# vladiant/CascadeClassifier

Measured on AMD Instinct MI355X. Metric: detection Mwindows/sec (1080p, haarcascade_frontalface) + achieved HBM GB/s, higher is better.
Workload: dtype i32+f32 (f64 stage sums)

## Files before the change

cascadeclassifier_amd/_lib.py:

```python
from __future__ import annotations

import ctypes as C
import os

_HERE = os.path.dirname(os.path.abspath(__file__))
LIB_PATH = os.environ.get("CCAMD_LIB") or os.path.join(_HERE, "lib", "libcascadeclassifier_amd.so")

CC_OK = 0
CC_ERR_INVALID_ARG = -1
CC_ERR_NO_DEVICE = -2
CC_ERR_HIP = -3
CC_ERR_IO = -4
CC_ERR_PARSE = -5
CC_ERR_UNSUPPORTED = -6
CC_ERR_BUFFER_TOO_SMALL = -7
CC_ERR_OUT_OF_RANGE = -8
CC_ERR_NO_TRAIN_PARAMS = -9

CC_FEATURE_HAAR, CC_FEATURE_LBP, CC_FEATURE_HOG = 0, 1, 2
CC_PIX_GRAY8, CC_PIX_BGR8, CC_PIX_BGRA8, CC_PIX_RGB8, CC_PIX_RGBA8, CC_PIX_RGB8_PLANAR = 0, 1, 2, 3, 4, 5
CC_HAAR_BASIC, CC_HAAR_CORE, CC_HAAR_ALL = 0, 1, 2


class CascadeError(RuntimeError):
# ... 119 lines not shown
    "cc_detect_batch_device_only": (_i, [_vp, _vp, _i, _i, _i, _i, _sz, _sz, C.POINTER(DetectParams)]),
    "cc_detect_multiscale_fmt": (_i, [_vp, _vp, _i, _i, _sz, _i, C.POINTER(DetectParams), _vp, _i, C.POINTER(_i)]),
    "cc_detect_batch_fmt": (_i, [_vp, _vp, _i, _i, _i, _i, _sz, _sz, _i, C.POINTER(DetectParams), _vp, _i, _vp]),
    "cc_detect_batch_submit_fmt": (_i, [_vp, _vp, _i, _i, _i, _i, _sz, _sz, _i, C.POINTER(DetectParams), _pp]),
    "cc_detect_batch_to_device": (_i, [_vp, _vp, _i, _i, _i, _i, _sz, _sz, _i, C.POINTER(DetectParams), _vp, _i, _vp,
                                       C.POINTER(_i)]),
    "cc_detect_batch_levels_fmt": (_i, [_vp, _vp, _i, _i, _i, _i, _sz, _sz, _i, C.POINTER(DetectParams), _vp, _vp, _vp, _i, _vp]),
    "cc_detect_batch_to_device_levels": (_i, [_vp, _vp, _i, _i, _i, _i, _sz, _sz, _i, C.POINTER(DetectParams), _vp, _vp, _vp, _i,
                                              _vp, C.POINTER(_i)]),
    "cc_detect_multiscale_levels_fmt": (_i, [_vp, _vp, _i, _i, _sz, _i, C.POINTER(DetectParams), _vp, _vp, _vp, _i,
                                             C.POINTER(_i)]),
    "cc_to_gray_u8": (_i, [_i, _vp, _i, _i, _i, _sz, _vp, _sz]),
    "cc_detect_multiscale_levels": (_i, [_vp, _vp, _i, _i, _sz, C.POINTER(DetectParams), _vp, _vp, _vp, _i, C.POINTER(_i)]),
    "cc_detect_raw": (_i, [_vp, _vp, _i, _i, _sz, C.POINTER(DetectParams), _vp, _i, C.POINTER(_i)]),
    "cc_detect_debug_windows": (_i, [_vp, _vp, _i, _i, _sz, C.POINTER(DetectParams), _vp, _vp, _vp, C.c_int64,
                                     C.POINTER(C.c_int64)]),
    "cc_scale_plan": (_i, [_i, _i, _i, _i, C.POINTER(DetectParams), _vp, _i, C.POINTER(_i)]),
    "cc_detector_specialize": (_i, [_vp, _i]),
    "cc_detector_specialize_async": (_i, [_vp, _i]),
    "cc_detector_specialized_stages": (_i, [_vp]),
    "cc_cascade_compile_specialized": (_i, [_vp, _i, C.c_char_p, C.POINTER(C.c_size_t)]),
    "cc_detector_set_profiling": (_i, [_vp, _i]),
    "cc_detector_graph_active": (_i, [_vp]),
    "cc_detector_graph_captures": (C.c_int64, [_vp]),
    "cc_detector_get_timings": (_i, [_vp, C.POINTER(DetectorTimings), _i]),
    "cc_detector_candidate_capacity": (_i, [_vp]),
    "cc_integral_u8": (_i, [_i, _vp, _i, _i, _sz, _vp, _vp, _vp]),
    "cc_resize_linear_exact_u8": (_i, [_i, _vp, _i, _i, _sz, _vp, _i, _i, _sz]),
    "cc_debug_stream_dwords": (_i, [_i, _sz, _i, C.POINTER(C.c_uint32)]),
    "cc_debug_division_check": (_i, [_i, C.c_uint64, C.c_uint64, C.POINTER(C.c_uint64)]),
    "cc_debug_vnf_check": (_i, [_i, C.c_uint64, C.c_uint64, C.POINTER(C.c_uint64)]),
    "cc_debug_wave_int_tables": (_i, [_vp, _vp, _vp, _vp, _vp]),
    "cc_debug_spec_step1_plan": (_i, [_vp, _i, _i, _vp, _vp, _vp, _vp]),
    "cc_group_rectangles": (_i, [_vp, _i, _i, _d, _vp, _i, C.POINTER(_i)]),
    "cc_group_rectangles_device": (_i, [_i, _vp, _vp, _i, _i, _d, _vp, _i, _vp, C.POINTER(_i)]),
    "cc_group_rectangles_levels": (_i, [_vp, _vp, _vp, _i, _i, _d, _vp, _vp, _vp, _i, C.POINTER(_i)]),
    "cc_group_rectangles_device_levels": (_i, [_i, _vp, _vp, _vp, _vp, _i, _i, _d, _vp, _vp, _vp, _i, _vp, C.POINTER(_i)]),
    "cc_eval_create": (_i, [_i, _i, _i, _i, _i, _i, _pp]),
    "cc_eval_destroy": (None, [_vp]),
    "cc_eval_num_features": (_i, [_vp]),
    "cc_eval_max_cat_count": (_i, [_vp]),
    "cc_eval_feature_size": (_i, [_vp]),
    "cc_eval_feature_geometry": (_i, [_vp, _i, _vp, _vp, C.POINTER(_i)]),
    "cc_eval_set_image": (_i, [_vp, _vp, _sz, C.c_uint8, _i]),
    "cc_eval_set_images": (_i, [_vp, _vp, _i, _i, _vp]),
    "cc_eval_labels": (C.POINTER(C.c_float), [_vp]),
    "cc_eval_calc": (_i, [_vp, _i, _i, C.POINTER(C.c_float)]),
    "cc_eval_calc_list": (_i, [_vp, _vp, _i, _i, _vp]),
    "cc_eval_calc_batch": (_i, [_vp, _i, _i, _vp, _i, _vp, _i]),
    "cc_eval_calc_batch_device": (_i, [_vp, _i, _i, _vp, _i, _vp, _sz]),
    "cc_eval_calc_batch_sorted": (_i, [_vp, _i, _i, _i, _vp, _vp, _i]),
    "cc_eval_calc_custom_haar": (_i, [_vp, _vp, _i, _i, _vp, _i, _vp]),
    "cc_haar_feature_calc": (_i, [_i, _vp, _i, _i, _vp, _vp, _i, _i, _vp]),
    "cc_eval_get_sample": (_i, [_vp, _i, _vp, _vp, _vp]),
    "cc_eval_hog_feature_geometry": (_i, [_vp, _i, _vp]),
    "cc_eval_get_hog_sample": (_i, [_vp, _i, _vp, _vp]),
    "cc_debug_hog_bins": (_i, [_i, C.POINTER(C.c_int32), _vp, _vp]),
    "cc_debug_hog_lds": (_i, [_i, _i, C.POINTER(_i), C.POINTER(_i), C.POINTER(C.c_int64), C.POINTER(C.c_int64)]),
    "cc_eval_predict_cascade": (_i, [_vp, _vp, _vp, _i, _vp]),
    "cc_eval_last_kernel_ms": (_i, [_vp, C.POINTER(C.c_double)]),
    "cc_debug_eval_tile_samples": (_i, [_vp]),
    "cc_eval_presort": (_i, [_vp, _i]),
    "cc_eval_presort_range": (_i, [_vp, _i, _i, _i]),
    "cc_presort_plan": (_i, [_i, _i, _i, C.c_uint64, C.POINTER(_i), C.POINTER(_i), C.POINTER(C.c_uint64)]),
    "cc_eval_presort_split": (_i, [_vp, _i, _i, _i, _i, _i]),
    "cc_eval_table_bytes": (_i, [_vp, C.POINTER(C.c_uint64)]),
# ... 98 lines not shown
```

cascadeclassifier_amd/csrc/cc_eval_common.h:

```cpp
#ifndef CC_EVAL_COMMON_H
#define CC_EVAL_COMMON_H

constexpr int TILE_X = 64;
#ifndef CC_TILE_Y
#define CC_TILE_Y 8
#endif
#ifndef CC_EVAL_THREADS
#define CC_EVAL_THREADS 256
#endif
#ifndef CC_EVAL_MIN_WAVES_PER_EU
#define CC_EVAL_MIN_WAVES_PER_EU 5
#endif
constexpr int TILE_Y = CC_TILE_Y;
constexpr int EVAL_THREADS = CC_EVAL_THREADS;
constexpr int EVAL_WAVES = EVAL_THREADS / 64;
constexpr int WIN_PER_THREAD = TILE_Y / EVAL_WAVES;
constexpr int SPEC_PARTS = EVAL_WAVES >= 8 ? 8 : EVAL_WAVES >= 4 ? 4 : EVAL_WAVES >= 2 ? 2 : 1;

struct ScaleDev {
  int w, h;
  int pitch8, pitchI;
  long long img_ofs, int_ofs, mask_ofs, win_ofs, h_ofs;
  int ystep, nx, ny, nxw, nbands;
  float scale;
  int win_w, win_h;
  int xtab_ofs, ytab_ofs;
};

struct HaarStumpDev {
  int ofs[3][4];
  float w[3];
  float thr, left, right;
  int nrect;
  int pad;
};
struct LbpStumpDev {
  int ofs[16];
  float left, right;
  int subset[8];
  int pad[2];
};

struct HaarNodeDev {
  int ofs[3][4];
  float w[3];
  float thr;
  int left, right;
  int nrect;
  int pad;
// ... 36 lines not shown

struct TileGeom16 {
  static constexpr bool k16 = true;
  int cols, rows, rs16, row_stride;
  __host__ __device__ TileGeom16(int W0, int H0, int tile_y = TILE_Y) {
    cols = (TILE_X - 1) * 2 + W0 + 1;
    rows = (tile_y - 1) * 2 + H0 + 1;
    rs16 = (cols + 3) / 4 * 4;
    if (rs16 % 16 == 0) rs16 += 4;
    row_stride = rs16 / 2;
  }
  __host__ __device__ int at(int r, int c) const { return r * rs16 + c; }
  __host__ __device__ int words() const { return rows * row_stride; }
};

constexpr int TILE_WINDOWS = TILE_X * TILE_Y;
constexpr int MAX_STAGES = 64;
constexpr int PART_DOUBLES = (EVAL_WAVES - 1) * 64;
constexpr int QUEUE_ROWS = TILE_WINDOWS / 32;
constexpr int VNF_PITCH = TILE_X + 32;
__host__ __device__ inline int tile_words_padded(int tile_words) { return (tile_words + 3) & ~3; }
__host__ __device__ inline size_t eval_lds_bytes(int tile_words, bool tilted, bool haar = true, int tile_y = TILE_Y, bool lean = false) {
  if (lean) return (size_t)tile_words_padded(tile_words) * 4 + tile_y * TILE_X * 4 + 2 * (tile_y * TILE_X) * 2 + 3 * 32 * 4;
  return (size_t)tile_words_padded(tile_words) * 4 * (tilted ? 2 : 1) + PART_DOUBLES * 8 + (haar ? tile_y * VNF_PITCH * 4 : 0) +
         2 * (tile_y * TILE_X) * 2 + 3 * 32 * 4;
}
__host__ __device__ inline int lean_split_gap_bytes(int tile_y, int rows) { return 2 * (tile_y * TILE_X) * 2 - 2 * rows * 32 * 2; }
__host__ __device__ inline int split_part_bytes(int ns) { return (ns - 1) * (EVAL_THREADS / ns) * 8; }
constexpr int CU_LDS_BYTES = 160 * 1024;
__host__ __device__ inline int lds_blocks_per_cu(size_t lds_bytes) {
  const int n = (int)((size_t)CU_LDS_BYTES / (lds_bytes ? lds_bytes : 1)), cap = 32 / EVAL_WAVES;
  return n > cap ? cap : n;
}

template <int CTRL, int ROW_MASK>
__device__ __forceinline__ double dpp_f64(double v) {
  const unsigned long long u = __double_as_longlong(v);
  const int lo = __builtin_amdgcn_update_dpp(0, (int)(unsigned)u, CTRL, ROW_MASK, 0xF, false);
  const int hi = __builtin_amdgcn_update_dpp(0, (int)(unsigned)(u >> 32), CTRL, ROW_MASK, 0xF, false);
  return __longlong_as_double(((unsigned long long)(unsigned)hi << 32) | (unsigned)lo);
}
__device__ __forceinline__ double readlane_f64(double v, int src) {
  const unsigned long long u = __double_as_longlong(v);
  const unsigned lo = __builtin_amdgcn_readlane((int)(unsigned)u, src);
  const unsigned hi = __builtin_amdgcn_readlane((int)(unsigned)(u >> 32), src);
  return __longlong_as_double(((unsigned long long)hi << 32) | lo);
}
__device__ __forceinline__ double wave_sum_f64(double v) {
  v += dpp_f64<0xB1, 0xF>(v);
  v += dpp_f64<0x4E, 0xF>(v);
  v += dpp_f64<0x141, 0xF>(v);
  v += dpp_f64<0x140, 0xF>(v);
  v += dpp_f64<0x142, 0xA>(v);
  v += dpp_f64<0x143, 0xC>(v);
  return readlane_f64(v, 63);
}
__device__ __forceinline__ int lane_rank(unsigned long long mask) {
  return __builtin_amdgcn_mbcnt_hi((unsigned)(mask >> 32), __builtin_amdgcn_mbcnt_lo((unsigned)mask, 0));
}

#endif
```

cascadeclassifier_amd/csrc/cc_eval_kernel.inc:

```

#define CC_CONST __attribute__((address_space(4)))
template <class T>
__device__ __forceinline__ const T CC_CONST* as_const_table(const T* p) {
  return (const T CC_CONST*)p;
}
template <class T>
__device__ __forceinline__ T load_record(const T CC_CONST* p) {
  static_assert(sizeof(T) % 4 == 0, "table records are dword multiples");
  T out;
  const int CC_CONST* w = (const int CC_CONST*)p;
  int* o = reinterpret_cast<int*>(&out);
#pragma unroll
  for (unsigned i = 0; i < sizeof(T) / 4; i++) o[i] = w[i];
  return out;
}

constexpr int STAGE_ROWS = 12;
template <int STEP, class Geom>
__device__ __forceinline__ void stage_tile(int32_t* lds, const Geom& G, const int32_t* __restrict__ sum,
                                           const ScaleDev& S, int x0, int y0) {
  const int lane = threadIdx.x & 63, wave = __builtin_amdgcn_readfirstlane(threadIdx.x >> 6);
  const int quads = (G.cols + 3) >> 2;
  const bool right_edge = x0 + quads * 4 - 1 > S.w;
  for (int q0 = 0; q0 < quads; q0 += 64) {
// ... 245 lines not shown

struct QueueState {
  int qg = 1;
  int st = 1;
  int n = 0, rows = 0, my_rows = 0;
};
struct WaveShare {
  int cnt, my_id;
  unsigned long long alive;
};

template <int STEP, bool HAAR, bool TREES>
struct EvalTile {
  using Stump = typename cc_select<HAAR, HaarStumpDev, LbpStumpDev>::type;
  using Node = typename cc_select<HAAR, HaarNodeDev, LbpNodeDev>::type;
#ifdef CC_SPEC_TILE16
  static constexpr bool G16 = STEP == 2 && !TREES;
#else
  static constexpr bool G16 = false;
#endif
  using Geom = typename cc_select<G16, TileGeom16, TileGeom<STEP>>::type;

  const EvalArgs& A;
  int32_t* const lds;
  const int4 T;
  const ScaleDev& S;
#ifdef CC_SPEC_W0
  static constexpr int W0 = CC_SPEC_W0, H0 = CC_SPEC_H0;
#else
  const int W0 = A.W0, H0 = A.H0;
#endif
  const Geom G{W0, H0};
#ifdef CC_LEAN_LDS
  static constexpr bool kLean = HAAR && !TREES && STEP == 1;
#else
  static constexpr bool kLean = false;
#endif
  double* const s_part = kLean ? nullptr : reinterpret_cast<double*>(lds + tile_words_padded(G.words()) * ((HAAR && A.tilt_chan >= 0) ? 2 : 1));
  float* const s_vnf = kLean ? reinterpret_cast<float*>(lds + tile_words_padded(G.words())) : reinterpret_cast<float*>(s_part + PART_DOUBLES);
  unsigned short* const s_q = reinterpret_cast<unsigned short*>(s_vnf + (HAAR ? TILE_Y * (kLean ? TILE_X : VNF_PITCH) : 0));
  int* const s_cnt = reinterpret_cast<int*>(s_q + 2 * TILE_WINDOWS);
  const int frame = blockIdx.y;
  const int32_t* const sum = A.integ + ((size_t)frame * A.nchan + 0) * A.int_frame_elems + S.int_ofs;
  const int lane = threadIdx.x & 63, wave = __builtin_amdgcn_readfirstlane(threadIdx.x >> 6);
  const int half = lane >> 5, cls = lane & 31;
  const int gx0 = T.y * TILE_X, gy0 = T.z * TILE_Y;
  const int skew = (STEP * G.row_stride) & 31;
  const Node* const nodes = reinterpret_cast<const Node*>(STEP == 2 ? A.nodes2 : A.nodes1);
  const Stump CC_CONST* const stumps = as_const_table(reinterpret_cast<const Stump*>(G16 ? A.gstumps : STEP == 2 ? A.stumps2 : A.stumps1));
  const int CC_CONST* const stage_first = as_const_table(A.stage_first);
  const int CC_CONST* const stage_ntrees = as_const_table(A.stage_ntrees);
  const float CC_CONST* const stage_thr = as_const_table(A.stage_thr);
  const int CC_CONST* const group_first = as_const_table(A.group_first);
  const double CC_CONST* const wave_q = as_const_table(A.wave_q);
  const int CC_CONST* const wave_thr_q = as_const_table(A.wave_thr_q);
  const bool dbg = A.dbg_codes != nullptr && frame == 0;

  __device__ __forceinline__ EvalTile(const EvalArgs& A_, int32_t* lds_, const int4 T_, const ScaleDev& S_) : A(A_), lds(lds_), T(T_), S(S_) {}

  __device__ __forceinline__ void stamp(int slot) const {
    if (A.stamps && threadIdx.x == 0)
      A.stamps[((size_t)blockIdx.y * gridDim.x + blockIdx.x) * STAMP_SLOTS + slot] = __builtin_amdgcn_s_memtime();
  }
  __device__ __forceinline__ int window_base(int id) const { return ((id >> 6) * STEP) * G.row_stride + (id & 63); }
  __device__ __forceinline__ auto table_reader(int id) const {
    if constexpr (G16)
      return GlobalReader{sum, (unsigned)((gy0 + (id >> 6)) * STEP) * (unsigned)S.pitchI + (unsigned)((gx0 + (id & 63)) * STEP), S.pitchI};
    else
      return LdsReader{lds + window_base(id)};
  }
  __device__ __forceinline__ void report(int id, int code, double last) const {
    const size_t o = (size_t)S.win_ofs + (size_t)(gy0 + (id >> 6)) * S.nx + (gx0 + (id & 63));
    A.dbg_codes[o] = code;
    if (A.dbg_sums) A.dbg_sums[o] = last;
  }
  __device__ __forceinline__ void emit_candidate(int id, double last_sum) const {
    const int slot = atomicAdd(A.cand_count, 1);
    if (slot < A.cand_cap) A.cands[slot] = CandRaw{frame, T.x, gx0 + (id & 63), gy0 + (id >> 6), last_sum};
  }
  __device__ __forceinline__ int win_class(int id) const { return ((id & 63) + skew * (id >> 6)) & 31; }
  __device__ __forceinline__ int vnf_slot(int id) const {
    if constexpr (kLean)
      return (id & ~63) | (((id & 63) + skew * (id >> 6)) & 63);
    else
      return (id >> 6) * (TILE_X + skew) + (id & 63);
  }
  __device__ __forceinline__ int q_index(int g, int row, int c) const {
    if constexpr (kLean)
      return (g & 1) ? (2 * QUEUE_ROWS - 1 - row) * 32 + c : row * 32 + c;
    else
      return (g & 1) * TILE_WINDOWS + row * 32 + c;
  }
// ... 100 lines not shown
        for (int j = lo; j < nt; j += step) {
          const Stump nxt = load_record(stumps + first + min(j + step, nt - 1));
          acc += stump_vote(rd, cur, vnf);
          cur = nxt;
        }
      }
    } else {
      for (int j = lo; j < nt; j += step) acc += stump_vote(rd, stumps + first + j, vnf);
    }
    return acc;
  }
  __device__ __forceinline__ WaveShare deal_windows(const QueueState& h) const {
    const unsigned short* q = s_q + (h.qg & 1) * TILE_WINDOWS;
    unsigned short* my_list = wave_lists(h.qg) + wave * 64;
    int numbered = 0;
    for (int r0 = 0; r0 < h.rows; r0 += 2) {
      const int row = r0 + half;
      const bool valid = row < h.my_rows;
      const int id = valid ? queued(q, h.qg, row, cls) : 0;
      const unsigned long long mask = __ballot(valid);
      const int number = numbered + lane_rank(mask);
      if (valid && number % EVAL_WAVES == wave) my_list[number / EVAL_WAVES] = (unsigned short)id;
      numbered += __builtin_popcountll(mask);
    }
    const int cnt = (numbered - wave + EVAL_WAVES - 1) / EVAL_WAVES;
    return WaveShare{cnt, lane < cnt ? my_list[lane] : 0, cnt >= 64 ? ~0ull : ((1ull << cnt) - 1ull)};
  }

  __device__ __forceinline__ void stage_phase(unsigned (&valsq_pre)[WIN_PER_THREAD]) const {
    unsigned sq_raw[WIN_PER_THREAD][4];
#pragma unroll
    for (int k = 0; k < WIN_PER_THREAD; k++) {
      sq_raw[k][0] = sq_raw[k][1] = sq_raw[k][2] = sq_raw[k][3] = 0;
      if (HAAR) {
        const int gx = min(gx0 + lane, S.nx - 1), gy = min(gy0 + wave * WIN_PER_THREAD + k, S.ny - 1);
        const unsigned* sq = reinterpret_cast<const unsigned*>(A.integ + ((size_t)frame * A.nchan + 1) * A.int_frame_elems + S.int_ofs);
        const int nrx = W0 - 2, nry = H0 - 2;
        size_t q0;
        int dx;
        if (STEP == 2 && A.sq_compact) {
          q0 = (size_t)(gy * 2 + 1) * S.pitchI + gx;
          dx = nrx >> 1;
        } else {
          q0 = (size_t)(gy * STEP + 1) * S.pitchI + (gx * STEP + 1);
          dx = nrx;
        }
        sq_raw[k][0] = sq[q0];
        sq_raw[k][1] = sq[q0 + dx];
        sq_raw[k][2] = sq[q0 + (size_t)nry * S.pitchI];
        sq_raw[k][3] = sq[q0 + (size_t)nry * S.pitchI + dx];
      }
    }
#ifdef CC_PRIO_STAGE
    __builtin_amdgcn_s_setprio(CC_PRIO_STAGE);
#endif
    stage_tile<STEP>(lds, G, sum, S, gx0 * STEP, gy0 * STEP);
    if (HAAR && A.tilt_chan >= 0)
      stage_tile<STEP>(lds + tile_words_padded(G.words()), G,
                       A.integ + ((size_t)frame * A.nchan + A.tilt_chan) * A.int_frame_elems + S.int_ofs, S, gx0 * STEP, gy0 * STEP);
    if (threadIdx.x < 3 * 32) s_cnt[threadIdx.x] = 0;
#pragma unroll
    for (int k = 0; k < WIN_PER_THREAD; k++) valsq_pre[k] = sq_raw[k][0] - sq_raw[k][1] - sq_raw[k][2] + sq_raw[k][3];
    __syncthreads();
#ifdef CC_PRIO_STAGE
    __builtin_amdgcn_s_setprio(0);
#endif
  }

  static constexpr bool kRolledDense = !HAAR && !TREES && WIN_PER_THREAD > 2;
  __device__ __forceinline__ void dense_phase_rolled() const {
    const int gx = gx0 + lane;
    const double thr0 = (double)stage_thr[0];
    unsigned long long* const mask_col = mask_column();
    [[maybe_unused]] const int nt0 = stage_ntrees[0];
#pragma unroll 1
    for (int k = 0; k < WIN_PER_THREAD; k++) {
      const int ly = wave * WIN_PER_THREAD + k;
      const int32_t* b = lds + (ly * STEP) * G.row_stride + lane;
      const bool alive = gx < S.nx && gy0 + ly < S.ny;
      double acc = 0.;
      if (__any(alive)) {
#ifdef CC_SPEC_STAGES
        acc = spec_stage<STEP>(0, 0, SPEC_PARTS, b, 1.f);
#else
        for (int i = 0; i < nt0; i++) acc += stump_vote(LdsReader{b}, stumps + i, 1.f);
#endif
      }
      deliver(stage0_outcome(ly, alive, acc, thr0, mask_col), ly * 64 + lane, acc, A.nstages == 1, 1);
    }
  }
  __device__ __forceinline__ bool dense_phase(const unsigned (&valsq_pre)[WIN_PER_THREAD]) const {
    int base[WIN_PER_THREAD];
    float vnf[WIN_PER_THREAD];
    bool alive[WIN_PER_THREAD];
    const int gx = gx0 + lane;
#pragma unroll
    for (int k = 0; k < WIN_PER_THREAD; k++) {
      const int ly = wave * WIN_PER_THREAD + k;
      const int gy = gy0 + ly;
      base[k] = (ly * STEP) * G.row_stride + lane;
      vnf[k] = 1.f;
      alive[k] = gx < S.nx && gy < S.ny;
      if (HAAR) {
        const bool in_grid = alive[k];
        alive[k] = false;
        if (in_grid) {
          const int nrx = W0 - 2, nry = H0 - 2;
          const double area = (double)(nrx * nry);
          const int32_t* b = lds + base[k];
          int valsum;
          if constexpr (G16) {
            const unsigned short* h = reinterpret_cast<const unsigned short*>(b);
            const int hx = nrx >> 1;
            const unsigned a0 = h[G.at(1, 1)], a1 = h[G.at(1, 1 + hx)], a2 = h[G.at(1, 1 + nrx)];
            const unsigned c0 = h[G.at(1 + nry, 1)], c1 = h[G.at(1 + nry, 1 + hx)], c2 = h[G.at(1 + nry, 1 + nrx)];
            valsum = (int)(((a0 - a1 - c0 + c1) & 0xffffu) + ((a1 - a2 - c1 + c2) & 0xffffu));
          } else
            valsum = b[G.at(1, 1)] - b[G.at(1, 1 + nrx)] - b[G.at(1 + nry, 1)] + b[G.at(1 + nry, 1 + nrx)];
          const unsigned valsq = valsq_pre[k];
          double nf = area * (double)valsq - (double)valsum * (double)valsum;
          if (nf > 0.) {
            vnf[k] = inv_sqrt_as_float(nf);
            alive[k] = area * (double)vnf[k] < 1e-1;
          }
          if (dbg && !alive[k]) report(ly * 64 + lane, -1, 0.0);
        }
      }
    }
    if (A.stop_after == -3) {
      float sink = 0;
#pragma unroll
      for (int k = 0; k < WIN_PER_THREAD; k++) sink += alive[k] ? vnf[k] : 0.f;
      if (HAAR && sink == 12345.f) s_vnf[0] = sink;
      return false;
    }
    bool any_mine = false;
    double acc[WIN_PER_THREAD];
#pragma unroll
    for (int k = 0; k < WIN_PER_THREAD; k++) {
      any_mine |= alive[k];
      acc[k] = 0.;
    }
    if (__any(any_mine)) {
      [[maybe_unused]] const int nt = stage_ntrees[0];
      if constexpr (TREES) {
        for (int i = 0; i < nt; i++) {
          const int root = as_const_table(A.tree_root)[i], leaf0 = as_const_table(A.tree_leaf0)[i];
#pragma unroll
          for (int k = 0; k < WIN_PER_THREAD; k++)
            if (alive[k]) acc[k] += tree_vote(lds + base[k], nodes, root, leaf0, A.leaves, vnf[k]);
        }
      } else {
#ifdef CC_SPEC_STAGES
        if constexpr (WIN_PER_THREAD == 2) {
          spec_stage0_x2<STEP>(lds + base[0], lds + base[1], vnf[0], vnf[1], acc[0], acc[1]);
        } else {
#pragma unroll
          for (int k = 0; k < WIN_PER_THREAD; k++) acc[k] = spec_stage<STEP>(0, 0, SPEC_PARTS, lds + base[k], vnf[k]);
        }
#else
        if constexpr (HAAR) {
          Stump cur = load_record(stumps);
          for (int i = 0; i < nt; i++) {
            const Stump nxt = load_record(stumps + min(i + 1, nt - 1));
#pragma unroll
            for (int k = 0; k < WIN_PER_THREAD; k++) acc[k] += stump_vote(LdsReader{lds + base[k]}, cur, vnf[k]);
            cur = nxt;
          }
        } else {
          for (int i = 0; i < nt; i++) {
#pragma unroll
            for (int k = 0; k < WIN_PER_THREAD; k++) acc[k] += stump_vote(LdsReader{lds + base[k]}, stumps + i, vnf[k]);
          }
        }
#endif
      }
    }
    const double thr = (double)stage_thr[0];
    unsigned long long* const mask_col = mask_column();
    bool pass_k[WIN_PER_THREAD];
#pragma unroll
    for (int k = 0; k < WIN_PER_THREAD; k++) pass_k[k] = stage0_outcome(wave * WIN_PER_THREAD + k, alive[k], acc[k], thr, mask_col);
    const bool last_group = A.nstages == 1;
#pragma unroll
    for (int k = 0; k < WIN_PER_THREAD; k++) {
      const int id = (wave * WIN_PER_THREAD + k) * 64 + lane;
      if (HAAR && pass_k[k] && !last_group) s_vnf[vnf_slot(id)] = vnf[k];
      deliver(pass_k[k], id, acc[k], last_group, 1);
    }
    return true;
  }

  __device__ __forceinline__ bool thread_phase(QueueState& h) const {
    for (; h.qg < A.ngroups; h.qg++) {
      const int qg = h.qg;
      const int st = h.st = group_first[qg];
      const int st_end = group_first[qg + 1];
      if (A.stop_after >= 0 && st > A.stop_after) return false;
      __syncthreads();
      if (qg >= A.dense_from) {
        h.n = min(s_cnt[(qg % 3) * 32], TILE_WINDOWS);
        h.rows = (h.n + 31) >> 5;
        h.my_rows = max(0, (h.n - cls + 31) >> 5);
      } else {
        h.my_rows = min(s_cnt[(qg % 3) * 32 + cls], QUEUE_ROWS);
        h.rows = wave_max_u32(h.my_rows);
        h.n = wave_sum_u32(h.my_rows) >> 1;
      }
      if (threadIdx.x < 32) s_cnt[((qg + 2) % 3) * 32 + threadIdx.x] = 0;
      if (st + 2 < STAMP_SLOTS - 1) stamp(st + 2);
      if (h.n == 0 || h.n < A.wave_below) break;
      const unsigned short* q = s_q + (qg & 1) * TILE_WINDOWS;
      const bool last_group = st_end >= A.nstages;
      const int groups = (h.rows + 1) >> 1;
      const bool may_split = A.split_stumps && st_end - st == 1;
      const int g_split = may_split ? groups - groups % EVAL_WAVES : groups;
      const int rem = groups - g_split;
      int ns = 1;
      if (rem > 0)
// ... 243 lines not shown
```

cascadeclassifier_amd/csrc/cc_spec.hip:

```cpp
#include <hip/hip_runtime.h>

#include <algorithm>
#include <array>
#include <cmath>
#include <cstdlib>
#include <cstring>
#include <map>
#include <mutex>

#include <dlfcn.h>
#include <sys/stat.h>
#include <unistd.h>

#include "cc_detect_internal.h"

namespace ccamd {

#include "build/cc_eval_kernel_src.h"

struct SpecStump {
  std::string loads;
  std::string decls;
  std::string compute;
  double base = 0.;
// ... 490 lines not shown
  bool ok() const { return create && compile && log_size && log && code_size && code && destroy; }
};

static const HipRtcApi& hiprtc_api() {
  static HipRtcApi api;
  static std::once_flag once;
  std::call_once(once, [] {
    for (const char* name : {"libhiprtc.so.7", "libhiprtc.so", "/opt/rocm/lib/libhiprtc.so"}) {
      api.lib = dlopen(name, RTLD_NOW | RTLD_LOCAL);
      if (api.lib) break;
    }
    if (!api.lib) return;
    auto sym = [&](const char* n) { return dlsym(api.lib, n); };
    api.create = reinterpret_cast<decltype(api.create)>(sym("hiprtcCreateProgram"));
    api.compile = reinterpret_cast<decltype(api.compile)>(sym("hiprtcCompileProgram"));
    api.log_size = reinterpret_cast<decltype(api.log_size)>(sym("hiprtcGetProgramLogSize"));
    api.log = reinterpret_cast<decltype(api.log)>(sym("hiprtcGetProgramLog"));
    api.code_size = reinterpret_cast<decltype(api.code_size)>(sym("hiprtcGetCodeSize"));
    api.code = reinterpret_cast<decltype(api.code)>(sym("hiprtcGetCode"));
    api.destroy = reinterpret_cast<decltype(api.destroy)>(sym("hiprtcDestroyProgram"));
    api.version = reinterpret_cast<decltype(api.version)>(sym("hiprtcVersion"));
  });
  return api;
}

static const char kSpecPrelude[] =
    "typedef signed char int8_t;\ntypedef unsigned char uint8_t;\ntypedef short int16_t;\ntypedef unsigned short uint16_t;\n"
    "typedef int int32_t;\ntypedef unsigned int uint32_t;\ntypedef long long int64_t;\ntypedef unsigned long long uint64_t;\n";

struct SpecModulePlan {
  int only_step, tile_y;
};
static bool spec_lean_lds(const Cascade& m, int tmode, int only_step) {
  return only_step == 1 && tmode == TILE_32 && m.feature_type == CC_FEATURE_HAAR && !m.has_tilted;
}
static size_t spec_step1_lds(const Cascade& m, int tile_y) {
  return eval_lds_bytes(TileGeom<1>(m.win_w, m.win_h, tile_y).words(), false, true, tile_y, true);
}
constexpr int kSpecStep1Rows = 20;
constexpr int kSpecStep1MinBlocks = 4;
static int spec_step1_rows(const Cascade& m, int want) {
  int ty = want;
  while (ty - EVAL_WAVES >= TILE_Y && lds_blocks_per_cu(spec_step1_lds(m, ty)) < kSpecStep1MinBlocks) ty -= EVAL_WAVES;
  return ty;
}
constexpr int kStep1WaveBelow = 32;
int spec_wave_below(int detector_value, int only_step, int tile_y) {
  if (only_step != 1 || detector_value <= 0) return -1;
  if (const char* e = std::getenv("CCAMD_WAVE_BELOW1")) return std::max(0, std::min(64, std::atoi(e)));
  if (std::getenv("CCAMD_WAVE_BELOW") || tile_y < 12) return -1;
  return std::max(detector_value, kStep1WaveBelow);
}

static std::vector<SpecModulePlan> spec_modules(const Cascade& m, int tmode) {
  auto valid = [&](int ty) { return ty >= EVAL_WAVES && ty <= 32 && ty % EVAL_WAVES == 0; };
  auto env_rows = [&](const char* name, int dflt) {
    const char* e = std::getenv(name);
    const int v = e ? std::atoi(e) : dflt;
    return valid(v) ? v : dflt;
  };
  if (m.has_tilted) return {{0, TILE_Y}};
  const bool lbp16 = m.feature_type == CC_FEATURE_LBP && tmode == TILE_16;
  const bool haar32 = tmode == TILE_32 && m.feature_type == CC_FEATURE_HAAR;
  const bool rows_given = std::getenv("CCAMD_SPEC_TILE_Y") != nullptr;
  const int all = env_rows("CCAMD_SPEC_TILE_Y", lbp16 ? 20 : TILE_Y);
  const bool two = (haar32 || std::getenv("CCAMD_SPEC_TWO_MODULES")) && !std::getenv("CCAMD_SPEC_ONE_MODULE");
  if (!two) return {{0, all}};
  return {{2, env_rows("CCAMD_SPEC_TILE_Y2", all)}, {1, env_rows("CCAMD_SPEC_TILE_Y1", (haar32 && !rows_given) ? spec_step1_rows(m, kSpecStep1Rows) : all)}};
}

static cc_status compile_specialised(const std::string& src, const std::string& arch, int n_stages, bool lbp, int tmode, int tile_y, int only_step, int win_w, int win_h,
                                     int lean_blocks, std::vector<char>& code) {
  const bool tile16 = tmode == TILE_16;
  static std::mutex mu;
  static std::map<std::string, std::vector<char>> cache;
  const std::string o_arch = "--offload-arch=" + arch, o_k = "-DCC_SPEC_STAGES=" + std::to_string(n_stages);
  const std::string o_ty = "-DCC_TILE_Y=" + std::to_string(tile_y), o_th = "-DCC_EVAL_THREADS=" + std::to_string(EVAL_THREADS);
  int min_waves = tile16 ? (tile_y >= 20 ? 6 : 7) : CC_EVAL_MIN_WAVES_PER_EU;
  if (lean_blocks > 0) {
    min_waves = std::max(1, std::min(8, lean_blocks * EVAL_WAVES / 4));
    if (const char* e = std::getenv("CCAMD_SPEC_WAVES1")) min_waves = std::max(1, std::min(8, std::atoi(e)));
  }
  const std::string o_w = "-DCC_EVAL_MIN_WAVES_PER_EU=" + std::to_string(min_waves);
  const std::string o_step = "-DCC_ONLY_STEP=" + std::to_string(only_step);
  const std::string o_w0 = "-DCC_SPEC_W0=" + std::to_string(win_w), o_h0 = "-DCC_SPEC_H0=" + std::to_string(win_h);
  std::vector<const char*> optv = {o_arch.c_str(), "-O3", "-std=c++17", "-ffp-contract=off", "-fno-fast-math", o_k.c_str(), o_ty.c_str(), o_th.c_str(), o_w.c_str(), o_w0.c_str(), o_h0.c_str()};
  if (only_step) optv.push_back(o_step.c_str());
  if (lbp) optv.push_back("-DCC_SPEC_LBP");
  if (tile16) optv.push_back("-DCC_SPEC_TILE16");
  if (lean_blocks > 0) optv.push_back("-DCC_LEAN_LDS");
  const char* const* opts = optv.data();
  const int n_opts = (int)optv.size();
  std::string key;
  {
    int major = 0, minor = 0;
    const HipRtcApi& rtc = hiprtc_api();
    if (rtc.version) (void)rtc.version(&major, &minor);
    key += "hiprtc " + std::to_string(major) + "." + std::to_string(minor) + " ";
  }
  for (int i = 0; i < n_opts; i++) key += std::string(opts[i]) + " ";
  key += "#" + src;
  {
    std::lock_guard<std::mutex> lk(mu);
    auto it = cache.find(key);
    if (it != cache.end()) {
      code = it->second;
      return CC_OK;
    }
  }
  struct CacheHeader {
    char magic[8];
    unsigned long long key_len, h1, h2;
  };
  auto hash_key = [&](unsigned long long seed, unsigned long long prime) {
// ... 81 lines not shown
      const bool ok = std::fwrite(&want, sizeof(want), 1, f) == 1 && std::fwrite(code.data(), 1, code.size(), f) == code.size();
      std::fclose(f);
      if (!ok || std::rename(tmp.c_str(), cache_file.c_str()) != 0) (void)std::remove(tmp.c_str());
    }
  }
  std::lock_guard<std::mutex> lk(mu);
  cache[key] = code;
  return CC_OK;
}

cc_status spec_build(const Cascade& m, int n_stages, const std::string& arch, std::vector<SpecCode>& codes, int& k_out, int& tmode_out) {
  if (cc_status hs = refuse_hog(m, "cc_detector_specialize"); hs != CC_OK) return hs;
  if (m.max_nodes_per_tree > 1) return set_error(CC_ERR_UNSUPPORTED, "cc_detector_specialize: stump cascades only");
  int k = 0, stumps = 0;
  const int budget = 320;
  while (k < (int)m.stage_ntrees.size() && k < n_stages && k < MAX_STAGES && (k == 0 || stumps + m.stage_ntrees[(size_t)k] <= budget))
    stumps += m.stage_ntrees[(size_t)k++];
  std::string src = kSpecPrelude;
  src += "namespace ccamd {\n";
  src += kEvalKernelSrc;
  src += "\n}  // namespace ccamd\n";
  const std::string marker = "//@@CC_SPEC_FUNCTIONS@@";
  const size_t pos = src.find(marker);
  if (pos == std::string::npos) return set_error(CC_ERR_HIP, "cc_detector_specialize: kernel source has no specialisation marker");
  const int tmode = tile16_eligible(m, k) ? TILE_16 : TILE_32;
  src.replace(pos, marker.size(), spec_stage_source(m, k, tmode));
  k_out = k;
  tmode_out = tmode;
  codes.clear();
  for (const SpecModulePlan& mp : spec_modules(m, tmode)) {
    SpecCode c;
    c.only_step = mp.only_step;
    c.tile_y = mp.tile_y;
    const int lean_blocks = spec_lean_lds(m, tmode, mp.only_step) ? std::max(1, lds_blocks_per_cu(spec_step1_lds(m, mp.tile_y))) : 0;
    const cc_status st = compile_specialised(src, arch, k, m.feature_type == CC_FEATURE_LBP, tmode, mp.tile_y, mp.only_step, m.win_w, m.win_h, lean_blocks, c.code);
    if (st != CC_OK) return st;
    codes.push_back(std::move(c));
  }
  return CC_OK;
}

cc_status spec_load(const Cascade& m, const std::vector<SpecCode>& codes, int tmode, size_t base_lds, SpecModule out[2], int* n_out) {
  if (codes.empty() || codes.size() > 2) return set_error(CC_ERR_HIP, "cc_detector_specialize: %zu modules", codes.size());
  const bool haar_k = m.feature_type == CC_FEATURE_HAAR;
  int n = 0;
  auto fail = [&](SpecModule& x) {
    (void)hipGetLastError();
    if (x.mod) (void)hipModuleUnload(x.mod);
    for (int i = 0; i < n; i++) (void)hipModuleUnload(out[i].mod);
  };
  for (const SpecCode& c : codes) {
    SpecModule x;
    x.tile_y = c.tile_y;
    x.only_step = c.only_step;
    const char* entry = c.only_step == 1 ? "k_eval_spec_step1" : c.only_step == 2 ? "k_eval_spec_step2" : "k_eval_spec";
    if (hipModuleLoadData(&x.mod, c.code.data()) != hipSuccess || hipModuleGetFunction(&x.fn, x.mod, entry) != hipSuccess) {
      fail(x);
      return set_error(CC_ERR_HIP, "cc_detector_specialize: the compiled module does not load or has no entry point");
    }
    const int ty = c.tile_y, step = c.only_step;
    x.lds = base_lds;
    if (tmode == TILE_32) {
      const TileGeom<1> G1(m.win_w, m.win_h, ty);
      const TileGeom<2> G2(m.win_w, m.win_h, ty);
      const int words = step == 1 ? G1.words() : step == 2 ? G2.words() : std::max(G1.words(), G2.words());
      x.lds = spec_lean_lds(m, tmode, step) ? spec_step1_lds(m, ty) : eval_lds_bytes(words, m.has_tilted, haar_k, ty);
    } else if (tmode == TILE_16) {
      const TileGeom<1> G1(m.win_w, m.win_h, ty);
      const TileGeom16 G2(m.win_w, m.win_h, ty);
      x.lds = eval_lds_bytes(std::max(G1.words(), G2.words()), false, haar_k, ty);
    }
    if (x.lds > 64 * 1024) {
      const hipError_t e = hipFuncSetAttribute(reinterpret_cast<const void*>(x.fn), hipFuncAttributeMaxDynamicSharedMemorySize, (int)x.lds);
      if (e != hipSuccess) {
        fail(x);
        return set_error(CC_ERR_UNSUPPORTED, "cc_detector_specialize: %zu bytes of LDS per tile cannot be requested for a run-time module (%s)",
                         x.lds, hipGetErrorString(e));
      }
    }
    if (std::getenv("CCAMD_TRACE_HOST")) {
      int nb = 0;
      if (hipModuleOccupancyMaxActiveBlocksPerMultiprocessor(&nb, x.fn, EVAL_THREADS, x.lds) != hipSuccess) (void)hipGetLastError();
      std::fprintf(stderr, "[ccamd host] specialised kernel: tile mode %d, tiles of step %d (0 = all), %d window rows, %zu bytes of LDS per block, %d resident blocks per CU\n",
                   tmode, c.only_step, ty, x.lds, nb);
    }
    out[n++] = x;
  }
  if (n == 2 && out[0].only_step == 1) std::swap(out[0], out[1]);
  *n_out = n;
  return CC_OK;
}

}

using namespace ccamd;

extern "C" {

cc_status cc_debug_spec_step1_plan(const cc_cascade* c, int rows_wanted, int wave_below_detector, int* rows, size_t* lds_bytes, int* blocks_per_cu,
                                   int* wave_below) {
  if (!c) return set_error(CC_ERR_INVALID_ARG, "cc_debug_spec_step1_plan: null cascade");
  if (cc_status hs = refuse_hog(c->m, "cc_debug_spec_step1_plan"); hs != CC_OK) return hs;
  if (c->m.max_nodes_per_tree > 1 || !spec_lean_lds(c->m, TILE_32, 1))
    return set_error(CC_ERR_UNSUPPORTED, "cc_debug_spec_step1_plan: upright Haar stump cascades only");
  const int ty = rows_wanted > 0 ? rows_wanted : spec_step1_rows(c->m, kSpecStep1Rows);
  if (ty < EVAL_WAVES || ty > 32 || ty % EVAL_WAVES) return set_error(CC_ERR_INVALID_ARG, "cc_debug_spec_step1_plan: %d window rows per tile", ty);
  const size_t lds = spec_step1_lds(c->m, ty);
  if (rows) *rows = ty;
  if (lds_bytes) *lds_bytes = lds;
  if (blocks_per_cu) *blocks_per_cu = lds_blocks_per_cu(lds);
  if (wave_below) {
    const int w = spec_wave_below(wave_below_detector, 1, ty);
    *wave_below = w >= 0 ? w : wave_below_detector;
  }
  return CC_OK;
}

cc_status cc_cascade_compile_specialized(const cc_cascade* c, int n_stages, const char* arch, size_t* code_bytes) {
  if (!c || !arch || !code_bytes) return set_error(CC_ERR_INVALID_ARG, "cc_cascade_compile_specialized: null argument");
  if (cc_status hs = refuse_hog(c->m, "cc_cascade_compile_specialized"); hs != CC_OK) return hs;
  std::vector<SpecCode> code;
  int k = 0;
  int tmode = 0;
  const cc_status st = spec_build(c->m, std::max(1, n_stages), arch, code, k, tmode);
  if (st != CC_OK) return st;
  *code_bytes = 0;
  for (const SpecCode& m : code) *code_bytes += m.code.size();
  return CC_OK;
}

}
```

include/cascadeclassifier_amd.h:

```cpp
#ifndef CASCADECLASSIFIER_AMD_H_
#define CASCADECLASSIFIER_AMD_H_

#include <stddef.h>
#include <stdint.h>

#ifdef __cplusplus
extern "C" {
#endif

#if defined(__GNUC__)
#define CC_API __attribute__((visibility("default")))
#else
#define CC_API
#endif

typedef int cc_status;
enum {
  CC_OK = 0,
  CC_ERR_INVALID_ARG = -1,
  CC_ERR_NO_DEVICE = -2,
  CC_ERR_HIP = -3,
  CC_ERR_IO = -4,
  CC_ERR_PARSE = -5,
  CC_ERR_UNSUPPORTED = -6,
// ... 130 lines not shown
CC_API int cc_detector_specialized_stages(const cc_detector* d);
CC_API cc_status cc_cascade_compile_specialized(const cc_cascade* c, int n_stages, const char* arch, size_t* code_bytes);

typedef struct cc_detector_timings {
  double resize_ms, integral_ms, eval_ms, finalize_ms;
  int64_t resize_launches, integral_launches, eval_launches, finalize_launches;
  int64_t frames;
  int64_t grid_windows;
  int64_t integral_elems;
  double eval_step1_ms;
  double group_ms;
  int64_t group_launches;
} cc_detector_timings;
CC_API cc_status cc_detector_set_profiling(cc_detector* d, int enabled);
CC_API int cc_detector_candidate_capacity(const cc_detector* d);
CC_API cc_status cc_detector_get_timings(cc_detector* d, cc_detector_timings* t, int reset);
CC_API int cc_detector_graph_active(const cc_detector* d);
CC_API int64_t cc_detector_graph_captures(const cc_detector* d);

CC_API cc_status cc_integral_u8(int device, const uint8_t* img, int width, int height, size_t row_stride, int32_t* sum,
                                int32_t* sqsum, int32_t* tilted);
CC_API cc_status cc_resize_linear_exact_u8(int device, const uint8_t* src, int sw, int sh, size_t sstride, uint8_t* dst,
                                           int dw, int dh, size_t dstride);
CC_API cc_status cc_resize_area_u8(int device, const uint8_t* src, int w, int h, size_t stride, uint8_t* dst, int dw, int dh);
CC_API cc_status cc_warp_perspective_u8(int device, const uint8_t* src, int sw, int sh, size_t sstride, uint8_t* dst, int dw,
                                        int dh, size_t dstride, const double* quad);
CC_API cc_status cc_to_gray_u8(int device, const uint8_t* src, int pixel_format, int width, int height, size_t row_stride,
                               uint8_t* dst, size_t dst_stride);
CC_API cc_status cc_debug_stream_dwords(int device, size_t n_bytes, int repeats, uint32_t* checksum);
CC_API cc_status cc_debug_division_check(int device, uint64_t n_pairs, uint64_t seed, uint64_t* mismatches);
CC_API cc_status cc_debug_vnf_check(int device, uint64_t n_values, uint64_t seed, uint64_t* mismatches);
CC_API cc_status cc_debug_wave_int_tables(const cc_cascade* c, double* q, int32_t* thr_q, int32_t* left_q, int32_t* right_q);
CC_API cc_status cc_debug_spec_step1_plan(const cc_cascade* c, int rows_wanted, int wave_below_detector, int* rows, size_t* lds_bytes,
                                          int* blocks_per_cu, int* wave_below);
CC_API cc_status cc_group_rectangles(const cc_rect* rects, int n, int group_threshold, double eps, cc_rect* out, int cap,
                                     int* n_out);
CC_API cc_status cc_group_rectangles_device(int device, const cc_rect* rects, const int32_t* offsets, int n_frames,
                                            int group_threshold, double eps, cc_rect* out, int cap, int32_t* out_offsets,
                                            int* n_total);
CC_API cc_status cc_group_rectangles_levels(const cc_rect* rects, const int32_t* levels, const double* weights, int n,
                                            int group_threshold, double eps, cc_rect* out, int32_t* out_levels,
                                            double* out_weights, int cap, int* n_out);
CC_API cc_status cc_group_rectangles_device_levels(int device, const cc_rect* rects, const int32_t* levels,
                                                   const double* weights, const int32_t* offsets, int n_frames,
                                                   int group_threshold, double eps, cc_rect* out, int32_t* out_levels,
                                                   double* out_weights, int cap, int32_t* out_offsets, int* n_total);

typedef struct cc_evaluator cc_evaluator;
enum { CC_HAAR_BASIC = 0, CC_HAAR_CORE = 1, CC_HAAR_ALL = 2 };

CC_API cc_status cc_eval_create(int feature_type, int haar_mode, int win_w, int win_h, int max_samples, int device,
                                cc_evaluator** out);
CC_API void cc_eval_destroy(cc_evaluator* e);
CC_API int cc_eval_num_features(const cc_evaluator* e);
CC_API int cc_eval_max_cat_count(const cc_evaluator* e);
CC_API int cc_eval_feature_size(const cc_evaluator* e);
CC_API cc_status cc_eval_feature_geometry(const cc_evaluator* e, int fi, int32_t* rects, float* weights, int* tilted);
CC_API cc_status cc_eval_hog_feature_geometry(const cc_evaluator* e, int feature_idx, int32_t* cells);
CC_API cc_status cc_eval_set_image(cc_evaluator* e, const uint8_t* img, size_t row_stride, uint8_t cls_label, int idx);
CC_API cc_status cc_eval_set_images(cc_evaluator* e, const uint8_t* imgs, int n, int first_idx, const uint8_t* labels);
CC_API const float* cc_eval_labels(const cc_evaluator* e);
CC_API cc_status cc_eval_calc(cc_evaluator* e, int fi, int si, float* out);
CC_API cc_status cc_eval_calc_list(cc_evaluator* e, const int32_t* feature_idx, int n_feats, int si, float* out);
CC_API cc_status cc_eval_calc_batch(cc_evaluator* e, int fi_begin, int fi_end, const int32_t* sample_idx, int n_samples,
                                    float* out, int out_on_device);
CC_API cc_status cc_eval_calc_batch_device(cc_evaluator* e, int fi_begin, int fi_end, const int32_t* sample_idx, int n_samples,
// ... 213 lines not shown
```

Baseline: 20130.

## Extend lean LDS layout to step-2 specialised kernel with taller ragged tiles

Enables the lean LDS layout for the step-2 specialised Haar module and picks a taller tile height that keeps the same number of resident blocks per CU, using an allocation-granularity-aware occupancy estimate. To allow tile heights that are not a multiple of the wave count, rows are now interleaved across waves, and a guard skips rows past the tile end. The aim is more window rows per block, meaning less integral-image halo reloaded per window, without losing occupancy. The cost is extra predication and unbalanced work across waves in ragged tiles.

```diff
diff --git a/cascadeclassifier_amd/_lib.py b/cascadeclassifier_amd/_lib.py
--- a/cascadeclassifier_amd/_lib.py
+++ b/cascadeclassifier_amd/_lib.py
@@ -175,6 +175,7 @@
     "cc_debug_vnf_check": (_i, [_i, C.c_uint64, C.c_uint64, C.POINTER(C.c_uint64)]),
     "cc_debug_wave_int_tables": (_i, [_vp, _vp, _vp, _vp, _vp]),
     "cc_debug_spec_step1_plan": (_i, [_vp, _i, _i, _vp, _vp, _vp, _vp]),
+    "cc_debug_spec_step2_plan": (_i, [_vp, _i, _i, _vp, _vp, _vp, _vp]),
     "cc_group_rectangles": (_i, [_vp, _i, _i, _d, _vp, _i, C.POINTER(_i)]),
     "cc_group_rectangles_device": (_i, [_i, _vp, _vp, _i, _i, _d, _vp, _i, _vp, C.POINTER(_i)]),
     "cc_group_rectangles_levels": (_i, [_vp, _vp, _vp, _i, _i, _d, _vp, _vp, _vp, _i, C.POINTER(_i)]),
diff --git a/cascadeclassifier_amd/csrc/cc_eval_common.h b/cascadeclassifier_amd/csrc/cc_eval_common.h
--- a/cascadeclassifier_amd/csrc/cc_eval_common.h
+++ b/cascadeclassifier_amd/csrc/cc_eval_common.h
@@ -14,7 +14,8 @@
 constexpr int TILE_Y = CC_TILE_Y;
 constexpr int EVAL_THREADS = CC_EVAL_THREADS;
 constexpr int EVAL_WAVES = EVAL_THREADS / 64;
-constexpr int WIN_PER_THREAD = TILE_Y / EVAL_WAVES;
+constexpr int WIN_PER_THREAD = (TILE_Y + EVAL_WAVES - 1) / EVAL_WAVES;
+constexpr bool RAGGED_ROWS = TILE_Y % EVAL_WAVES != 0;
 constexpr int SPEC_PARTS = EVAL_WAVES >= 8 ? 8 : EVAL_WAVES >= 4 ? 4 : EVAL_WAVES >= 2 ? 2 : 1;
 
 struct ScaleDev {
@@ -117,6 +118,12 @@
   const int n = (int)((size_t)CU_LDS_BYTES / (lds_bytes ? lds_bytes : 1)), cap = 32 / EVAL_WAVES;
   return n > cap ? cap : n;
 }
+constexpr int LDS_ALLOC_BYTES = 1280;
+__host__ __device__ inline int lds_blocks_resident(size_t lds_bytes) {
+  const size_t units = (lds_bytes + LDS_ALLOC_BYTES - 1) / LDS_ALLOC_BYTES;
+  const int n = (int)((size_t)(CU_LDS_BYTES / LDS_ALLOC_BYTES) / (units ? units : 1)), cap = 32 / EVAL_WAVES;
+  return n > cap ? cap : n;
+}
 
 template <int CTRL, int ROW_MASK>
 __device__ __forceinline__ double dpp_f64(double v) {
diff --git a/cascadeclassifier_amd/csrc/cc_eval_kernel.inc b/cascadeclassifier_amd/csrc/cc_eval_kernel.inc
--- a/cascadeclassifier_amd/csrc/cc_eval_kernel.inc
+++ b/cascadeclassifier_amd/csrc/cc_eval_kernel.inc
@@ -301,7 +301,7 @@
 #endif
   const Geom G{W0, H0};
 #ifdef CC_LEAN_LDS
-  static constexpr bool kLean = HAAR && !TREES && STEP == 1;
+  static constexpr bool kLean = HAAR && !TREES;
 #else
   static constexpr bool kLean = false;
 #endif
@@ -327,6 +327,8 @@
 
   __device__ __forceinline__ EvalTile(const EvalArgs& A_, int32_t* lds_, const int4 T_, const ScaleDev& S_) : A(A_), lds(lds_), T(T_), S(S_) {}
 
+  __device__ __forceinline__ int own_row(int k) const { return RAGGED_ROWS ? wave + k * EVAL_WAVES : wave * WIN_PER_THREAD + k; }
+  __device__ __forceinline__ bool has_row(int k) const { return !RAGGED_ROWS || k < WIN_PER_THREAD - 1 || own_row(k) < TILE_Y; }
   __device__ __forceinline__ void stamp(int slot) const {
     if (A.stamps && threadIdx.x == 0)
       A.stamps[((size_t)blockIdx.y * gridDim.x + blockIdx.x) * STAMP_SLOTS + slot] = __builtin_amdgcn_s_memtime();
@@ -493,8 +495,8 @@
 #pragma unroll
     for (int k = 0; k < WIN_PER_THREAD; k++) {
       sq_raw[k][0] = sq_raw[k][1] = sq_raw[k][2] = sq_raw[k][3] = 0;
-      if (HAAR) {
-        const int gx = min(gx0 + lane, S.nx - 1), gy = min(gy0 + wave * WIN_PER_THREAD + k, S.ny - 1);
+      if (HAAR && has_row(k)) {
+        const int gx = min(gx0 + lane, S.nx - 1), gy = min(gy0 + own_row(k), S.ny - 1);
         const unsigned* sq = reinterpret_cast<const unsigned*>(A.integ + ((size_t)frame * A.nchan + 1) * A.int_frame_elems + S.int_ofs);
         const int nrx = W0 - 2, nry = H0 - 2;
         size_t q0;
@@ -536,7 +538,8 @@
     [[maybe_unused]] const int nt0 = stage_ntrees[0];
 #pragma unroll 1
     for (int k = 0; k < WIN_PER_THREAD; k++) {
-      const int ly = wave * WIN_PER_THREAD + k;
+      if (!has_row(k)) continue;
+      const int ly = own_row(k);
       const int32_t* b = lds + (ly * STEP) * G.row_stride + lane;
       const bool alive = gx < S.nx && gy0 + ly < S.ny;
       double acc = 0.;
@@ -557,11 +560,11 @@
     const int gx = gx0 + lane;
 #pragma unroll
     for (int k = 0; k < WIN_PER_THREAD; k++) {
-      const int ly = wave * WIN_PER_THREAD + k;
+      const int ly = own_row(k);
       const int gy = gy0 + ly;
       base[k] = (ly * STEP) * G.row_stride + lane;
       vnf[k] = 1.f;
-      alive[k] = gx < S.nx && gy < S.ny;
+      alive[k] = has_row(k) && gx < S.nx && gy < S.ny;
       if (HAAR) {
         const bool in_grid = alive[k];
         alive[k] = false;
@@ -613,11 +616,12 @@
         }
       } else {
 #ifdef CC_SPEC_STAGES
-        if constexpr (WIN_PER_THREAD == 2) {
+        if constexpr (WIN_PER_THREAD == 2 && !RAGGED_ROWS) {
           spec_stage0_x2<STEP>(lds + base[0], lds + base[1], vnf[0], vnf[1], acc[0], acc[1]);
         } else {
 #pragma unroll
-          for (int k = 0; k < WIN_PER_THREAD; k++) acc[k] = spec_stage<STEP>(0, 0, SPEC_PARTS, lds + base[k], vnf[k]);
+          for (int k = 0; k < WIN_PER_THREAD; k++)
+            if (has_row(k)) acc[k] = spec_stage<STEP>(0, 0, SPEC_PARTS, lds + base[k], vnf[k]);
         }
 #else
         if constexpr (HAAR) {
@@ -625,13 +629,15 @@
           for (int i = 0; i < nt; i++) {
             const Stump nxt = load_record(stumps + min(i + 1, nt - 1));
 #pragma unroll
-            for (int k = 0; k < WIN_PER_THREAD; k++) acc[k] += stump_vote(LdsReader{lds + base[k]}, cur, vnf[k]);
+            for (int k = 0; k < WIN_PER_THREAD; k++)
+              if (has_row(k)) acc[k] += stump_vote(LdsReader{lds + base[k]}, cur, vnf[k]);
             cur = nxt;
           }
         } else {
           for (int i = 0; i < nt; i++) {
 #pragma unroll
-            for (int k = 0; k < WIN_PER_THREAD; k++) acc[k] += stump_vote(LdsReader{lds + base[k]}, stumps + i, vnf[k]);
+            for (int k = 0; k < WIN_PER_THREAD; k++)
+              if (has_row(k)) acc[k] += stump_vote(LdsReader{lds + base[k]}, stumps + i, vnf[k]);
           }
         }
 #endif
@@ -641,11 +647,13 @@
     unsigned long long* const mask_col = mask_column();
     bool pass_k[WIN_PER_THREAD];
 #pragma unroll
-    for (int k = 0; k < WIN_PER_THREAD; k++) pass_k[k] = stage0_outcome(wave * WIN_PER_THREAD + k, alive[k], acc[k], thr, mask_col);
+    for (int k = 0; k < WIN_PER_THREAD; k++)
+      pass_k[k] = has_row(k) && stage0_outcome(own_row(k), alive[k], acc[k], thr, mask_col);
     const bool last_group = A.nstages == 1;
 #pragma unroll
     for (int k = 0; k < WIN_PER_THREAD; k++) {
-      const int id = (wave * WIN_PER_THREAD + k) * 64 + lane;
+      if (!has_row(k)) continue;
+      const int id = own_row(k) * 64 + lane;
       if (HAAR && pass_k[k] && !last_group) s_vnf[vnf_slot(id)] = vnf[k];
       deliver(pass_k[k], id, acc[k], last_group, 1);
     }
diff --git a/cascadeclassifier_amd/csrc/cc_spec.hip b/cascadeclassifier_amd/csrc/cc_spec.hip
--- a/cascadeclassifier_amd/csrc/cc_spec.hip
+++ b/cascadeclassifier_amd/csrc/cc_spec.hip
@@ -546,10 +546,16 @@
   int only_step, tile_y;
 };
 static bool spec_lean_lds(const Cascade& m, int tmode, int only_step) {
-  return only_step == 1 && tmode == TILE_32 && m.feature_type == CC_FEATURE_HAAR && !m.has_tilted;
+  return (only_step == 1 || only_step == 2) && tmode == TILE_32 && m.feature_type == CC_FEATURE_HAAR && !m.has_tilted;
 }
 static size_t spec_step1_lds(const Cascade& m, int tile_y) {
   return eval_lds_bytes(TileGeom<1>(m.win_w, m.win_h, tile_y).words(), false, true, tile_y, true);
+}
+static size_t spec_step2_lds(const Cascade& m, int tile_y) {
+  return eval_lds_bytes(TileGeom<2>(m.win_w, m.win_h, tile_y).words(), false, true, tile_y, true);
+}
+static size_t spec_lean_request(const Cascade& m, int only_step, int tile_y) {
+  return only_step == 2 ? spec_step2_lds(m, tile_y) : spec_step1_lds(m, tile_y);
 }
 constexpr int kSpecStep1Rows = 20;
 constexpr int kSpecStep1MinBlocks = 4;
@@ -558,20 +564,34 @@
   while (ty - EVAL_WAVES >= TILE_Y && lds_blocks_per_cu(spec_step1_lds(m, ty)) < kSpecStep1MinBlocks) ty -= EVAL_WAVES;
   return ty;
 }
+constexpr int kSpecStep2MaxRows = 12;
+static int spec_step2_rows(const Cascade& m) {
+  const int blocks = lds_blocks_resident(spec_step2_lds(m, TILE_Y));
+  if (blocks < 1) return TILE_Y;
+  int ty = TILE_Y;
+  while (ty + 1 <= kSpecStep2MaxRows && lds_blocks_resident(spec_step2_lds(m, ty + 1)) >= blocks) ty++;
+  return ty;
+}
+static int spec_lean_blocks(const Cascade& m, int only_step, int tile_y) {
+  return only_step == 2 ? lds_blocks_resident(spec_step2_lds(m, tile_y)) : lds_blocks_per_cu(spec_step1_lds(m, tile_y));
+}
 constexpr int kStep1WaveBelow = 32;
 int spec_wave_below(int detector_value, int only_step, int tile_y) {
-  if (only_step != 1 || detector_value <= 0) return -1;
-  if (const char* e = std::getenv("CCAMD_WAVE_BELOW1")) return std::max(0, std::min(64, std::atoi(e)));
+  if ((only_step != 1 && only_step != 2) || detector_value <= 0) return -1;
+  if (const char* e = std::getenv(only_step == 1 ? "CCAMD_WAVE_BELOW1" : "CCAMD_WAVE_BELOW2")) return std::max(0, std::min(64, std::atoi(e)));
+  if (only_step == 2) return -1;
   if (std::getenv("CCAMD_WAVE_BELOW") || tile_y < 12) return -1;
   return std::max(detector_value, kStep1WaveBelow);
 }
 
 static std::vector<SpecModulePlan> spec_modules(const Cascade& m, int tmode) {
-  auto valid = [&](int ty) { return ty >= EVAL_WAVES && ty <= 32 && ty % EVAL_WAVES == 0; };
-  auto env_rows = [&](const char* name, int dflt) {
+  auto valid = [&](int ty, bool any_height) {
+    return any_height ? ty >= TILE_Y && ty <= kSpecStep2MaxRows : ty >= EVAL_WAVES && ty <= 32 && ty % EVAL_WAVES == 0;
+  };
+  auto env_rows = [&](const char* name, int dflt, bool any_height = false) {
     const char* e = std::getenv(name);
     const int v = e ? std::atoi(e) : dflt;
-    return valid(v) ? v : dflt;
+    return valid(v, any_height) ? v : dflt;
   };
   if (m.has_tilted) return {{0, TILE_Y}};
   const bool lbp16 = m.feature_type == CC_FEATURE_LBP && tmode == TILE_16;
@@ -580,7 +600,8 @@
   const int all = env_rows("CCAMD_SPEC_TILE_Y", lbp16 ? 20 : TILE_Y);
   const bool two = (haar32 || std::getenv("CCAMD_SPEC_TWO_MODULES")) && !std::getenv("CCAMD_SPEC_ONE_MODULE");
   if (!two) return {{0, all}};
-  return {{2, env_rows("CCAMD_SPEC_TILE_Y2", all)}, {1, env_rows("CCAMD_SPEC_TILE_Y1", (haar32 && !rows_given) ? spec_step1_rows(m, kSpecStep1Rows) : all)}};
+  const bool lean2 = spec_lean_lds(m, tmode, 2);
+  return {{2, env_rows("CCAMD_SPEC_TILE_Y2", (lean2 && !rows_given) ? spec_step2_rows(m) : all, lean2)}, {1, env_rows("CCAMD_SPEC_TILE_Y1", (haar32 && !rows_given) ? spec_step1_rows(m, kSpecStep1Rows) : all)}};
 }
 
 static cc_status compile_specialised(const std::string& src, const std::string& arch, int n_stages, bool lbp, int tmode, int tile_y, int only_step, int win_w, int win_h,
@@ -593,7 +614,7 @@
   int min_waves = tile16 ? (tile_y >= 20 ? 6 : 7) : CC_EVAL_MIN_WAVES_PER_EU;
   if (lean_blocks > 0) {
     min_waves = std::max(1, std::min(8, lean_blocks * EVAL_WAVES / 4));
-    if (const char* e = std::getenv("CCAMD_SPEC_WAVES1")) min_waves = std::max(1, std::min(8, std::atoi(e)));
+    if (const char* e = only_step == 1 ? std::getenv("CCAMD_SPEC_WAVES1") : nullptr) min_waves = std::max(1, std::min(8, std::atoi(e)));
   }
   const std::string o_w = "-DCC_EVAL_MIN_WAVES_PER_EU=" + std::to_string(min_waves);
   const std::string o_step = "-DCC_ONLY_STEP=" + std::to_string(only_step);
@@ -741,7 +762,7 @@
     SpecCode c;
     c.only_step = mp.only_step;
     c.tile_y = mp.tile_y;
-    const int lean_blocks = spec_lean_lds(m, tmode, mp.only_step) ? std::max(1, lds_blocks_per_cu(spec_step1_lds(m, mp.tile_y))) : 0;
+    const int lean_blocks = spec_lean_lds(m, tmode, mp.only_step) ? std::max(1, spec_lean_blocks(m, mp.only_step, mp.tile_y)) : 0;
     const cc_status st = compile_specialised(src, arch, k, m.feature_type == CC_FEATURE_LBP, tmode, mp.tile_y, mp.only_step, m.win_w, m.win_h, lean_blocks, c.code);
     if (st != CC_OK) return st;
     codes.push_back(std::move(c));
@@ -773,7 +794,7 @@
       const TileGeom<1> G1(m.win_w, m.win_h, ty);
       const TileGeom<2> G2(m.win_w, m.win_h, ty);
       const int words = step == 1 ? G1.words() : step == 2 ? G2.words() : std::max(G1.words(), G2.words());
-      x.lds = spec_lean_lds(m, tmode, step) ? spec_step1_lds(m, ty) : eval_lds_bytes(words, m.has_tilted, haar_k, ty);
+      x.lds = spec_lean_lds(m, tmode, step) ? spec_lean_request(m, step, ty) : eval_lds_bytes(words, m.has_tilted, haar_k, ty);
     } else if (tmode == TILE_16) {
       const TileGeom<1> G1(m.win_w, m.win_h, ty);
       const TileGeom16 G2(m.win_w, m.win_h, ty);
@@ -788,10 +809,11 @@
       }
     }
     if (std::getenv("CCAMD_TRACE_HOST")) {
-      int nb = 0;
+      int nb = 0, scratch = -1;
       if (hipModuleOccupancyMaxActiveBlocksPerMultiprocessor(&nb, x.fn, EVAL_THREADS, x.lds) != hipSuccess) (void)hipGetLastError();
-      std::fprintf(stderr, "[ccamd host] specialised kernel: tile mode %d, tiles of step %d (0 = all), %d window rows, %zu bytes of LDS per block, %d resident blocks per CU\n",
-                   tmode, c.only_step, ty, x.lds, nb);
+      if (hipFuncGetAttribute(&scratch, HIP_FUNC_ATTRIBUTE_LOCAL_SIZE_BYTES, x.fn) != hipSuccess) (void)hipGetLastError();
+      std::fprintf(stderr, "[ccamd host] specialised kernel: tile mode %d, tiles of step %d (0 = all), %d window rows, %zu bytes of LDS per block, %d resident blocks per CU, %d bytes of scratch per lane\n",
+                   tmode, c.only_step, ty, x.lds, nb, scratch);
     }
     out[n++] = x;
   }
@@ -825,6 +847,25 @@
   return CC_OK;
 }
 
+cc_status cc_debug_spec_step2_plan(const cc_cascade* c, int rows_wanted, int wave_below_detector, int* rows, size_t* lds_bytes, int* blocks_per_cu,
+                                   int* wave_below) {
+  if (!c) return set_error(CC_ERR_INVALID_ARG, "cc_debug_spec_step2_plan: null cascade");
+  if (cc_status hs = refuse_hog(c->m, "cc_debug_spec_step2_plan"); hs != CC_OK) return hs;
+  if (c->m.max_nodes_per_tree > 1 || !spec_lean_lds(c->m, TILE_32, 2))
+    return set_error(CC_ERR_UNSUPPORTED, "cc_debug_spec_step2_plan: upright Haar stump cascades only");
+  const int ty = rows_wanted > 0 ? rows_wanted : spec_step2_rows(c->m);
+  if (ty < TILE_Y || ty > kSpecStep2MaxRows) return set_error(CC_ERR_INVALID_ARG, "cc_debug_spec_step2_plan: %d window rows per tile", ty);
+  const size_t lds = spec_step2_lds(c->m, ty);
+  if (rows) *rows = ty;
+  if (lds_bytes) *lds_bytes = lds;
+  if (blocks_per_cu) *blocks_per_cu = lds_blocks_resident(lds);
+  if (wave_below) {
+    const int w = spec_wave_below(wave_below_detector, 2, ty);
+    *wave_below = w >= 0 ? w : wave_below_detector;
+  }
+  return CC_OK;
+}
+
 cc_status cc_cascade_compile_specialized(const cc_cascade* c, int n_stages, const char* arch, size_t* code_bytes) {
   if (!c || !arch || !code_bytes) return set_error(CC_ERR_INVALID_ARG, "cc_cascade_compile_specialized: null argument");
   if (cc_status hs = refuse_hog(c->m, "cc_cascade_compile_specialized"); hs != CC_OK) return hs;
diff --git a/include/cascadeclassifier_amd.h b/include/cascadeclassifier_amd.h
--- a/include/cascadeclassifier_amd.h
+++ b/include/cascadeclassifier_amd.h
@@ -186,6 +186,8 @@
 CC_API cc_status cc_debug_vnf_check(int device, uint64_t n_values, uint64_t seed, uint64_t* mismatches);
 CC_API cc_status cc_debug_wave_int_tables(const cc_cascade* c, double* q, int32_t* thr_q, int32_t* left_q, int32_t* right_q);
 CC_API cc_status cc_debug_spec_step1_plan(const cc_cascade* c, int rows_wanted, int wave_below_detector, int* rows, size_t* lds_bytes,
+                                          int* blocks_per_cu, int* wave_below);
+CC_API cc_status cc_debug_spec_step2_plan(const cc_cascade* c, int rows_wanted, int wave_below_detector, int* rows, size_t* lds_bytes,
                                           int* blocks_per_cu, int* wave_below);
 CC_API cc_status cc_group_rectangles(const cc_rect* rects, int n, int group_threshold, double eps, cc_rect* out, int cap,
                                      int* n_out);
```

After: 20670 (median of 6 runs). +2.7%, better.
